# satoutahhaithem/gym

Measured on AMD Instinct MI355X. Metric: strategy-step param GB/s (%HBM/xGMI peak) + ms/outer step, GPT-2 124M, 1-8 GPUs, higher is better.
Workload: dtype f32

## Files before the change

### gym_amd/_lib.py

```python
import ctypes
import os
import threading

_HERE = os.path.dirname(os.path.abspath(__file__))
LIB_PATH = os.environ.get("GYM_AMD_LIB") or os.path.join(_HERE, "_lib", "libgym_amd.so")
HEADER_PATH = os.path.join(os.path.dirname(_HERE), "include", "gym_amd.h")

GA_F32 = 0
GA_BF16 = 1
GA_BF16_REF = 2
GA_LAYOUT_ROWS = 0
GA_LAYOUT_ELEM_MAJOR = 1
GA_MASK_BYTES = 0
GA_MASK_BITS = 1
GA_MASK_TORCH = 2

c_i32, c_i64, c_u32, c_u64, c_f32, c_f64 = (ctypes.c_int32, ctypes.c_int64, ctypes.c_uint32,
                                            ctypes.c_uint64, ctypes.c_float, ctypes.c_double)
c_p = ctypes.c_void_p


class TorchDraw(ctypes.Structure):
    _fields_ = [("table", c_p), ("ntens", c_i32), ("p", c_f32), ("seed", c_u64), ("offset0", c_u64),
                ("offset_step", c_u64), ("seedoff", c_p)]


class DemoTensor(ctypes.Structure):
    _fields_ = [
        ("offset", c_i64), ("payload_off", c_i64),
        ("rows", c_i32), ("cols", c_i32),
        ("n1", c_i32), ("n2", c_i32),
        ("gy", c_i32), ("gx", c_i32),
        ("k", c_i32),
        ("basis1", c_i32), ("basis2", c_i32),
        ("chunk_start", c_i32),
    ]


class DemoRowGroup(ctypes.Structure):
    _fields_ = [("offset", c_i64), ("payload_off", c_i64), ("rows", c_i32), ("k", c_i32)]


SIGNATURES = {
    "ga_abi_version": (c_i32, []),
    "ga_last_error": (ctypes.c_char_p, []),
    "ga_stream_copy": (c_i32, [c_p, c_p, c_i64, c_p]),
    "ga_probe_random_words": (c_i32, [c_p, c_i64, c_i64, c_p, c_i64, c_i32, c_p]),
    "ga_probe_philox": (c_i32, [c_i64, c_p, c_p]),
    "ga_probe_chunk_stream": (c_i32, [c_p, c_p, c_i64, c_i64, c_i32, c_p]),
    "ga_probe_diloco_placement": (c_i32, [c_p, c_i64, c_i64, c_i64, c_p, c_p, c_p]),
    "ga_probe_mean_placement": (c_i32, [c_p, c_i64, c_i64, c_i64, c_p]),
    "ga_probe_adam_placement": (c_i32, [c_p, c_p, c_p, c_p, c_i64, c_i64, c_i64, c_p]),
    "ga_replica_mean": (c_i32, [c_i32, c_p, c_i64, c_i64, c_p, c_i64, c_f32, c_p, c_i64, c_i64, c_p]),
    "ga_diloco_outer": (c_i32, [c_i32, c_p, c_i64, c_i64, c_i64, c_f32, c_p, c_p, c_i32, c_i32, c_f32, c_f32,
                                c_f32, c_f32, c_i32, c_p, c_i64, c_i64, c_p]),
    "ga_diloco_outer_masked": (c_i32, [c_i32, c_p, c_i64, c_i64, c_i64, c_p, c_f32, c_f32, c_p, c_p, c_i32, c_i32,
                                       c_f32, c_f32, c_f32, c_f32, c_i32, c_p, c_i64, c_i64, c_p]),
    "ga_sparta_workspace_bytes": (c_i64, [c_i64]),
    "ga_sparta_gap_table": (None, [c_f64, c_p]),
    "ga_sparta_pack_mask": (c_i32, [c_p, c_i64, c_p, c_p]),
    "ga_sparta_torch_bernoulli_span": (c_i64, []),
    "ga_sparta_torch_draw_bytes": (c_i32, []),
    "ga_sparta_torch_bernoulli": (c_i32, [c_p, c_i32, c_i64, c_f32, c_u64, c_u64, c_u64, c_p, c_p, c_i32, c_p]),
    "ga_sparta_select": (c_i32, [c_i32, c_p, c_i64, c_i64, c_i32, c_i64, c_p, c_i32, c_u64, c_u64, c_f64, c_p, c_i64,
                                 c_i64, c_p, c_p, c_p, c_p, c_p]),
    "ga_sparta_scatter": (c_i32, [c_i32, c_p, c_p, c_p, c_i64, c_f32, c_p, c_i64, c_i64, c_i32, c_p]),
    "ga_sparta_average_local": (c_i32, [c_i32, c_p, c_i64, c_i64, c_i32, c_i64, c_p, c_i32, c_u64, c_u64, c_f64, c_p,
                                        c_i64, c_f32, c_p, c_p, c_i64, c_p, c_p, c_p]),
    "ga_demo_tensor_bytes": (c_i32, []),
    "ga_demo_encode": (c_i32, [c_i32, c_p, c_i32, c_i32, c_p, c_p, c_p, c_p, c_p, c_i64, c_i64, c_f32, c_f32,
                               c_f32, c_p, c_i64, c_i64, c_p]),
    "ga_demo_encode_sym": (c_i32, [c_i32, c_p, c_i32, c_i32, c_p, c_i32, c_p, c_p, c_p, c_p, c_i64, c_i64,
                                   c_f32, c_f32, c_f32, c_p, c_i64, c_i64, c_p]),
    "ga_demo_decode": (c_i32, [c_i32, c_p, c_i32, c_i32, c_p, c_p, c_i64, c_i64, c_i64, c_p, c_p, c_i64,
                               c_i64, c_f32, c_p]),
    "ga_demo_decode_sym": (c_i32, [c_i32, c_p, c_i32, c_i32, c_p, c_i32, c_p, c_p, c_i64, c_i64, c_i64, c_p, c_p,
                                   c_i64, c_i64, c_f32, c_p]),
    "ga_sumsq_partials_count": (c_i32, []),
    "ga_grad_clip_coef": (c_i32, [c_i32, c_p, c_i64, c_i64, c_i64, c_f32, c_p, c_p, c_p]),
    "ga_adam_step": (c_i32, [c_i32, c_p, c_p, c_p, c_p, c_i64, c_i64, c_i64, c_f32, c_f32, c_f32, c_f32, c_f32,
                             c_f32, c_f32, c_f32, c_p, c_p]),
    "ga_replica_gram_workspace_bytes": (c_i64, [c_i64, c_i64]),
    "ga_replica_gram_chain": (c_i32, []),
    "ga_replica_gram": (c_i32, [c_i32, c_p, c_i64, c_i64, c_i64, c_p, c_p, c_p, c_p, c_p]),
    "ga_replica_gram_centered_workspace_bytes": (c_i64, [c_i64, c_i64]),
    "ga_replica_gram_centered": (c_i32, [c_i32, c_p, c_i64, c_i64, c_i64, c_p, c_p, c_p, c_p, c_p, c_p]),
}

_lib = None
_lock = threading.Lock()


class HipLibraryError(RuntimeError):
    pass


def lib():
    global _lib
    if _lib is not None:
        return _lib
    with _lock:
        if _lib is None:
            if not os.path.exists(LIB_PATH):
                raise HipLibraryError(
                    f"{LIB_PATH} is not built: run `make` (or `python __graft_entry__.py`) in the repo root; "
                    "gym_amd has no CPU fallback")
            L = ctypes.CDLL(LIB_PATH)
            for name, (res, args) in SIGNATURES.items():
                fn = getattr(L, name)
                fn.restype = res
                fn.argtypes = args
            if L.ga_demo_tensor_bytes() != ctypes.sizeof(DemoTensor):
                raise HipLibraryError("ga_demo_tensor layout mismatch between libgym_amd.so and gym_amd/_lib.py")
            _lib = L
    return _lib


def check(rc, what):
    if rc != 0:
        msg = lib().ga_last_error().decode(errors="replace")
        raise HipLibraryError(f"{what} failed (code {rc}): {msg}")


def header_symbols(path=HEADER_PATH):
    import re
    txt = open(path).read()
    txt = re.sub(r"/\*.*?\*/", "", txt, flags=re.S)
    return re.findall(r"GA_API\s+[\w\s\*]+?\b(ga_\w+)\s*\(", txt)
```

### gym_amd/csrc/demo_wave.hip

```cpp
#include "ga_common.h"

namespace ga {
namespace dw {

constexpr int kWaves = 8;
constexpr int kThreads = 64 * kWaves;
constexpr int kLd = 65;
constexpr int kCand = 128;
static_assert(2 * (kCand + 64) >= 320, "the fallback top-k keeps its maps in lst[128..319]");

typedef float f32x16 __attribute__((ext_vector_type(16)));

#ifdef GA_DEMO_STAMPS
extern __device__ unsigned long long* g_demo_stamps_w;
#define DW_PH_DECL unsigned long long ph_acc[16] = {}, ph_last = __builtin_amdgcn_s_memtime()
#define DW_PH(i)                                                    \
    do {                                                            \
        const unsigned long long t_ = __builtin_amdgcn_s_memtime(); \
        ph_acc[i] += t_ - ph_last;                                  \
        ph_last = t_;                                               \
    } while (0)
#define DW_CNT(i) (ph_acc[i] += 1)
#define DW_PH_FLUSH()                                                                                       \
    do {                                                                                                    \
        if ((threadIdx.x & 63) == 0) {                                                                      \
            unsigned long long* row_ = g_demo_stamps_w + ((size_t)blockIdx.x * kWaves + (threadIdx.x >> 6)) * 16; \
            for (int i_ = 0; i_ < 16; ++i_) row_[i_] = ph_acc[i_];                                          \
        }                                                                                                   \
    } while (0)
#else
#define DW_PH_DECL do {} while (0)
#define DW_PH(i) do {} while (0)
#define DW_CNT(i) do {} while (0)
#define DW_PH_FLUSH() do {} while (0)
#endif

#define WAVE_LDS_SYNC() asm volatile("" ::: "memory")

__device__ __forceinline__ int lane_id() {
    int t = (int)threadIdx.x;
    asm volatile("" : "+v"(t));
    return t & 63;
}

__device__ __forceinline__ f32x16 zero16() {
    f32x16 a;
#pragma unroll
    for (int r = 0; r < 16; ++r) a[r] = 0.f;
    return a;
}

__device__ __forceinline__ f32x16 mfma(float a, float b, const f32x16& c) {
    return __builtin_amdgcn_mfma_f32_32x32x2f32(a, b, c, 0, 0, 0);
}

__device__ __forceinline__ constexpr int rowmap(int r, int h) { return (r & 3) + 8 * (r >> 2) + 4 * h; }

__device__ __forceinline__ int blk(int h, int q) { return h ? 4 + q : (q < 4 ? q : 8 + q); }

__device__ __forceinline__ int pi_col(int H, int m) { return 4 * blk((m >> 2) & 1, 4 * H + (m >> 3)) + (m & 3); }

__device__ __forceinline__ float basis64(const float* Hb, int i, int d) {
    const float v = Hb[(i < 32 ? i : 63 - i) * kLd + d];
    return (i >= 32 && (d & 1)) ? -v : v;
}

__device__ __forceinline__ uint32_t keyv(float v) { return (__float_as_uint(v) & 0x7fffffffu) + 1u; }

__device__ __forceinline__ int wave_excl_scan128(int v) {
    int r = 0;
#pragma unroll
    for (int b = 0; b < 7; ++b) {
        const uint64_t m = __ballot((v >> b) & 1);
        r += (int)__builtin_amdgcn_mbcnt_hi((uint32_t)(m >> 32), __builtin_amdgcn_mbcnt_lo((uint32_t)m, 0u)) << b;
    }
    return r;
}

__device__ __forceinline__ int wave_sum(int v) {
#pragma unroll
    for (int d = 32; d > 0; d >>= 1) v += __shfl_xor(v, d, 64);
    return v;
}

__device__ __forceinline__ int find_tensor(const ga_demo_tensor* __restrict__ T, int ntens, int tix, int chunk) {
    int lo = tix < 0 ? 0 : tix, hi = ntens - 1;
    while (lo < hi) {
        const int mid = (lo + hi + 1) >> 1;
        if (T[mid].chunk_start <= chunk) lo = mid;
        else hi = mid - 1;
    }
    return lo;
}

__device__ __forceinline__ void decode_wave_priority() {
    const int w = __builtin_amdgcn_readfirstlane((int)threadIdx.x >> 6);
    asm volatile("s_cmp_lt_u32 %0, 4\n\ts_cbranch_scc1 1f\n\ts_setprio 1\n1:" ::"s"(w) : "scc");
}

__device__ __forceinline__ uint32_t rdl(uint32_t v, int j) {
    return (uint32_t)__builtin_amdgcn_readlane((int)v, j);
}

struct ListLDS {
    uint32_t lst[2 * (kCand + 64)];
    uint32_t bm[128];
    uint32_t sm[4];
};

struct WaveLDS : ListLDS {
    float tile[64 * kLd];
};

__device__ __forceinline__ uint32_t lane_off(int s, int q, int l, int h, int stride) {
    return (uint32_t)((s ? 63 - l : l) * stride + 4 * blk(h, q));
}

template <typename T>
__device__ __forceinline__ const T* at_off(const T* pb, uint32_t off) {
    return reinterpret_cast<const T*>(reinterpret_cast<const char*>(pb) + (uint64_t)(uint32_t)(off * (uint32_t)sizeof(T)));
}
template <typename T>
__device__ __forceinline__ T* at_off(T* pb, uint32_t off) {
    return reinterpret_cast<T*>(reinterpret_cast<char*>(pb) + (uint64_t)(uint32_t)(off * (uint32_t)sizeof(T)));
}

template <typename T>
__device__ __forceinline__ void load_rows(const T* pb, int stride, int l, int h, bool vec, int nrows,
                                          float (&o)[2][8][4]) {
    if (vec && nrows == 64) {
#pragma unroll
        for (int s = 0; s < 2; ++s)
#pragma unroll
            for (int q = 0; q < 8; ++q)
                Vec4<T>::unpack(*reinterpret_cast<const typename Vec4<T>::type*>(at_off(pb, lane_off(s, q, l, h, stride))),
                                o[s][q]);
        return;
    }
#pragma unroll
    for (int s = 0; s < 2; ++s) {
        const bool live = (s ? 63 - l : l) < nrows;
#pragma unroll
        for (int q = 0; q < 8; ++q) {
            const T* a = at_off(pb, lane_off(s, q, l, h, stride));
            if (live && vec) {
                Vec4<T>::unpack(*reinterpret_cast<const typename Vec4<T>::type*>(a), o[s][q]);
            } else {
#pragma unroll
                for (int e = 0; e < 4; ++e) o[s][q][e] = live ? Elem<T>::load(a + e) : 0.f;
            }
        }
    }
}

template <typename T>
__device__ __forceinline__ void store_rows(T* pb, int stride, int l, int h, bool vec, int nrows,
                                           const float (&o)[2][8][4]) {
    if (vec && nrows == 64) {
#pragma unroll
        for (int s = 0; s < 2; ++s)
#pragma unroll
            for (int q = 0; q < 8; ++q)
                *reinterpret_cast<typename Vec4<T>::type*>(at_off(pb, lane_off(s, q, l, h, stride))) = Vec4<T>::pack(o[s][q]);
        return;
    }
#pragma unroll
    for (int s = 0; s < 2; ++s) {
        if ((s ? 63 - l : l) >= nrows) continue;
#pragma unroll
        for (int q = 0; q < 8; ++q) {
            T* a = at_off(pb, lane_off(s, q, l, h, stride));
            if (vec) {
                *reinterpret_cast<typename Vec4<T>::type*>(a) = Vec4<T>::pack(o[s][q]);
            } else {
#pragma unroll
                for (int e = 0; e < 4; ++e) Elem<T>::store(a + e, o[s][q][e]);
            }
        }
    }
}
// ... 552 lines not shown
    }
    DW_PH(6);
    {
        const int lane = lane_id(), l = lane & 31, h = lane >> 5;
        f32x16 Tm[2][2];
        row_product(x, Hb, l, h, Tm);
#pragma unroll
        for (int s = 0; s < 2; ++s)
#pragma unroll
            for (int qc = 0; qc < 2; ++qc)
#pragma unroll
                for (int r = 0; r < 16; ++r) {
                    const int i = rowmap(r, h);
                    W.tile[(s ? 63 - i : i) * kLd + 2 * l + qc] = Tm[s][qc][r];
                }
    }
    WAVE_LDS_SYNC();
    {
        const int L = lane_id();
        float* trow = W.tile + L * kLd;
        float yr[64];
#pragma unroll
        for (int t = 0; t < 64; ++t) yr[t] = trow[t];
        uint32_t thr = 0;
        for (int bit = 31; bit >= 0; --bit) {
            const uint32_t cnd = thr | (1u << bit);
            int cl = 0;
#pragma unroll
            for (int t = 0; t < 64; ++t) cl += fabsf(yr[t]) >= __uint_as_float(cnd - 1u) ? 1 : 0;
            if (cl >= k) thr = cnd;
        }
        int gl = 0;
#pragma unroll
        for (int t = 0; t < 64; ++t) gl += keyv(yr[t]) > thr ? 1 : 0;
        int need = k - gl;
        int slot = 0;
        const bool live = L < rows;
        int32_t* oi = pay_idx + (int64_t)L * k;
        float* ov = pay_val + (int64_t)L * k;
#pragma unroll
        for (int t = 0; t < 64; ++t) {
            const uint32_t kv = keyv(yr[t]);
            const bool tie = kv == thr && need > 0;
            const bool s = kv > thr || tie;
            need -= tie ? 1 : 0;
            if (s && live) {
                oi[slot] = t;
                ov[slot] = yr[t];
            }
            slot += s ? 1 : 0;
            trow[t] = s ? yr[t] : 0.f;
        }
    }
    WAVE_LDS_SYNC();
    {
        const int lane = lane_id(), l = lane & 31, h = lane >> 5;
        const int c0 = pi_col(0, l), c1 = pi_col(1, l);
#pragma unroll
        for (int s = 0; s < 2; ++s) {
            const float* yrow = W.tile + (s ? 63 - l : l) * kLd;
            f32x16 r0 = zero16(), r1 = zero16();
#pragma unroll
            for (int t = 0; t < 32; ++t) {
                const int d = 2 * t + h;
                const float yv = yrow[d];
                r0 = mfma(basis64(Hb, c0, d), yv, r0);
                r1 = mfma(basis64(Hb, c1, d), yv, r1);
            }
#pragma unroll
            for (int q = 0; q < 8; ++q)
#pragma unroll
                for (int e = 0; e < 4; ++e) x[s][q][e] -= (q < 4 ? r0 : r1)[4 * (q & 3) + e];
        }
        store_rows(delta, 64, l, h, vec, rows, x);
    }
    WAVE_LDS_SYNC();
    DW_PH(7);
}

template <typename T>
__global__ __launch_bounds__(kThreads) void encode_kernel(
    const ga_demo_tensor* __restrict__ tens, int ntens, int nchunks, const ga_demo_rowgroup* __restrict__ groups,
    int ngroups, const float* __restrict__ F64, T* param0, const T* __restrict__ grad0, T* delta0, int64_t ld,
    int64_t K, float lr, float decay, float wd_factor, int32_t* payload0, int64_t pstride, int64_t M, int ptr_vec) {
    __shared__ float Hb[32 * kLd];
    __shared__ WaveLDS wl[kWaves];
    __shared__ int next_job;
    for (int q = threadIdx.x; q < 32 * 64; q += kThreads) Hb[(q >> 6) * kLd + (q & 63)] = F64[q];
    next_job = 0;
    __syncthreads();
    const int wid = __builtin_amdgcn_readfirstlane((int)threadIdx.x >> 6);
    WaveLDS& W = wl[wid];
    DW_PH_DECL;
    const int64_t n64 = (int64_t)nchunks * K;
    const int64_t stride = (int64_t)gridDim.x * kWaves;
    const int64_t b8 = (int64_t)blockIdx.x * kWaves;
    const int64_t g_total = (int64_t)ngroups * K;
    const uint32_t st = (uint32_t)stride;
    uint32_t nc32 = 0;
#pragma unroll
    for (int w = 0; w < kWaves; ++w)
        if (b8 + w < n64) nc32 += ((uint32_t)(n64 - (b8 + w)) + st - 1u) / st;
    const int64_t nc = nc32;
    const int64_t ng = (int64_t)blockIdx.x < g_total
                           ? ((uint32_t)(g_total - blockIdx.x) + gridDim.x - 1u) / gridDim.x : 0;
    const int64_t nt = nc + ng;
    int tix = -1;
    int64_t last_rep = -1;
    while (true) {
        int tv = 0;
        if (lane_id() == 0) tv = atomicAdd(&next_job, 1);
        const int64_t t = __builtin_amdgcn_readfirstlane(tv);
        if (t >= nt) break;
        const int64_t job = t < ng ? n64 + (int64_t)blockIdx.x + t * gridDim.x
                                   : b8 + ((t - ng) & 7) + ((t - ng) >> 3) * stride;
        if (job < n64) {
            const int64_t rep = job / nchunks;
            const int chunk = (int)(job - rep * nchunks);
            if (rep != last_rep) {
                tix = -1;
                last_rep = rep;
            }
            tix = find_tensor(tens, ntens, tix, chunk);
            const ga_demo_tensor td = tens[tix];
            const int c = chunk - td.chunk_start;
            int32_t* pi = payload0 + rep * pstride + td.payload_off + (int64_t)c * td.k;
            float* pv = reinterpret_cast<float*>(payload0 + rep * pstride + M) + td.payload_off + (int64_t)c * td.k;
            chunk64<T>(td, c, param0 + rep * ld, grad0 + rep * ld, delta0 + rep * ld, pi, pv, lr, decay, wd_factor,
                       ptr_vec, Hb, W
#ifdef GA_DEMO_STAMPS
                       , ph_acc, ph_last
#endif
            );
            DW_CNT(9);
        } else {
            const int64_t j = job - n64;
            const int64_t rep = j / ngroups;
            const int g = (int)(j - rep * ngroups);
            const ga_demo_rowgroup rg = groups[g];
            rowgroup<T>(rg, param0 + rep * ld, grad0 + rep * ld, delta0 + rep * ld,
                        payload0 + rep * pstride + rg.payload_off,
                        reinterpret_cast<float*>(payload0 + rep * pstride + M) + rg.payload_off, lr, decay,
                        wd_factor, ptr_vec, Hb, W
#ifdef GA_DEMO_STAMPS
                        , ph_acc, ph_last
#endif
            );
        }
    }
    DW_PH_FLUSH();
}

template <typename T>
static int launch(const ga_demo_tensor* tens, int32_t ntens, int32_t nchunks, const ga_demo_rowgroup* groups,
                  int32_t ngroups, const float* F64, void* param, const void* grad, void* delta, int64_t K,
                  int64_t ld, float lr, float decay, float wd_factor, int32_t* payload, int64_t pstride, int64_t M,
                  int ptr_vec, hipStream_t stream) {
    static const int cus = [] {
        int dev = 0, n = 0;
        (void)hipGetDevice(&dev);
        (void)hipDeviceGetAttribute(&n, hipDeviceAttributeMultiprocessorCount, dev);
        return n > 0 ? n : 256;
    }();
    auto kern = encode_kernel<T>;
    static const int resident = [&] {
        int per_cu = 0;
        (void)hipOccupancyMaxActiveBlocksPerMultiprocessor(&per_cu, kern, kThreads, 0);
        return (per_cu > 0 ? per_cu : 1) * cus;
    }();
    const int64_t jobs = ((int64_t)nchunks + ngroups) * K;
    const int64_t want = (jobs + kWaves - 1) / kWaves;
    const int grid = (int)(want < resident ? want : resident);
    if (grid <= 0) return GA_OK;
    hipLaunchKernelGGL(kern, dim3(grid), dim3(kThreads), 0, stream, tens, ntens, nchunks, groups, ngroups, F64,
                       (T*)param, (const T*)grad, (T*)delta, ld, K, lr, decay, wd_factor, payload, pstride, M,
                       ptr_vec);
    return GA_OK;
}

constexpr int kMaxSrc = 15;

struct DecLDS {
    float tile[64 * 64];
    uint32_t aux[512];
};

__device__ __forceinline__ int fidx(int row, int col) { return row * 64 + 4 * ((col >> 2) ^ (row & 15)) + (col & 3); }

__device__ __forceinline__ float sgnf(float g) {
    return fabsf(g) > 0.f ? __builtin_copysignf(1.f, g) : 0.f;
}

template <typename T>
using PRaw = typename Vec4<T>::type[16];

template <typename T>
__device__ __forceinline__ void load_coal_raw(const T* pb, int stride, bool vec, int lane, PRaw<T>& o) {
    if (vec) {
#pragma unroll
        for (int i = 0; i < 16; ++i)
            o[i] = *reinterpret_cast<const typename Vec4<T>::type*>(at_off(pb, coal_off(i, lane, stride)));
    } else {
#pragma unroll
        for (int i = 0; i < 16; ++i) {
            float f[4];
#pragma unroll
            for (int e = 0; e < 4; ++e) f[e] = Elem<T>::load(at_off(pb, coal_off(i, lane, stride)) + e);
            o[i] = Vec4<T>::pack(f);
        }
    }
}

template <typename T, bool NTS = false>
__device__ __forceinline__ void store_quad(T* pb, int i, int stride, bool vec, int lane, const float (&f)[4]) {
    T* a = at_off(pb, coal_off(i, lane, stride));
    if (vec) {
        if constexpr (NTS) stream_store(reinterpret_cast<typename Vec4<T>::type*>(a), Vec4<T>::pack(f));
        else store_vec(pb, coal_off(i, lane, stride), Vec4<T>::pack(f));
    } else {
#pragma unroll
        for (int e = 0; e < 4; ++e) Elem<T>::store(a + e, f[e]);
    }
}

template <typename T, bool NTS = false>
__device__ __forceinline__ void sign_update(const float4* tile, T* pr, T* gr, int stride, bool vec, float lr,
                                            int lane, PRaw<T>& raw) {
    if constexpr (sizeof(typename Vec4<T>::type) < 16) {
#pragma unroll
        for (int i = 0; i < 16; ++i) {
            const float4 v = tile[t4((lane >> 4) + 4 * i, lane & 15)];
            float f[4];
            Vec4<T>::unpack(raw[i], f);
            f[0] = fmaf(-lr, v.x, f[0]);
            f[1] = fmaf(-lr, v.y, f[1]);
            f[2] = fmaf(-lr, v.z, f[2]);
            f[3] = fmaf(-lr, v.w, f[3]);
            store_quad(pr, i, stride, vec, lane, f);
        }
        if (gr) {
#pragma unroll
            for (int i = 0; i < 16; ++i) {
                const float4 v = tile[t4((lane >> 4) + 4 * i, lane & 15)];
                const float f[4] = {v.x, v.y, v.z, v.w};
                store_quad<T, NTS>(gr, i, stride, vec, lane, f);
            }
        }
    } else {
#pragma unroll
        for (int i = 0; i < 16; ++i) {
            const float4 v = tile[t4((lane >> 4) + 4 * i, lane & 15)];
            raw[i].x = fmaf(-lr, v.x, raw[i].x);
            raw[i].y = fmaf(-lr, v.y, raw[i].y);
            raw[i].z = fmaf(-lr, v.z, raw[i].z);
            raw[i].w = fmaf(-lr, v.w, raw[i].w);
        }
        if (vec) {
#pragma unroll
            for (int i = 0; i < 16; ++i) *reinterpret_cast<float4*>(at_off(pr, coal_off(i, lane, stride))) = raw[i];
        } else {
// ... 337 lines not shown
        PRaw<T> p0;
        tix = find_tensor(tens, ntens, tix, (int)job);
        ga_demo_tensor td = tens[tix];
        dchunk_entries(td, (int)job - td.chunk_start, payload, pstride, M, S, cur);
        dchunk_params<T>(td, (int)job - td.chunk_start, param, ptr_vec, p0);
        while (true) {
            const int c = (int)job - td.chunk_start;
            const int64_t base = chunk_base(td, c);
            const bool vec = chunk_vec(td, ptr_vec);
            const int cols = td.cols, kc = td.k;
            job += stride;
            if (job < nchunks) {
                tix = find_tensor(tens, ntens, tix, (int)job);
                td = tens[tix];
            }
            dchunk_signs(kc, S, cur, Hb, W, [&] {
                if (job < nchunks) dchunk_entries(td, (int)job - td.chunk_start, payload, pstride, M, S, cur);
            });
            apply_signs<T, NTS>(reinterpret_cast<const float4*>(W.tile), param + base, grad ? grad + base : nullptr,
                                K, ld, cols, vec, 64, lr, lane_id(), p0);
            WAVE_LDS_SYNC();
            if (job >= nchunks) break;
            dchunk_params<T>(td, (int)job - td.chunk_start, param, ptr_vec, p0);
        }
    }
    for (; job < total; job += stride) {
        const ga_demo_rowgroup rg = groups[(int)(job - nchunks)];
        dgroup<T>(rg, payload, pstride, M, S, param, grad, K, ld, lr, ptr_vec, Hb, W);
    }
}

template <typename T, int MS>
static void launch_decode_ms(const ga_demo_tensor* tens, int32_t ntens, int32_t nchunks,
                             const ga_demo_rowgroup* groups, int32_t ngroups, const float* F64,
                             const int32_t* payload, int64_t pstride, int64_t M, int S, void* param, void* grad,
                             int64_t K, int64_t ld, float lr, int ptr_vec, hipStream_t stream) {
    auto kern = decode_kernel<T, MS>;
    static const int resident = [&] {
        int per_cu = 0, dev = 0, cus = 0;
        (void)hipOccupancyMaxActiveBlocksPerMultiprocessor(&per_cu, kern, kThreads, 0);
        (void)hipGetDevice(&dev);
        (void)hipDeviceGetAttribute(&cus, hipDeviceAttributeMultiprocessorCount, dev);
        return (per_cu > 0 ? per_cu : 1) * (cus > 0 ? cus : 256);
    }();
    const int64_t jobs = (int64_t)nchunks + ngroups;
    const int64_t want = (jobs + kWaves - 1) / kWaves;
    const int64_t wr = (int64_t)kWaves * resident;
    int64_t m = S >= 2 ? (8 * jobs + 7 * wr) / (14 * wr)
                       : (6 * jobs + 16 * wr) / (32 * wr);
    if (m < 1) m = 1;
    const int64_t g = resident * m;
    const int grid = (int)(g < want ? g : want);
    if (grid <= 0) return;
    if (S >= 2)
        hipLaunchKernelGGL((decode_kernel<T, MS, true>), dim3(grid), dim3(kThreads), 0, stream, tens, ntens, nchunks,
                           groups, ngroups, F64, payload, pstride, M, S, (T*)param, (T*)grad, K, ld, lr, ptr_vec);
    else
        hipLaunchKernelGGL(kern, dim3(grid), dim3(kThreads), 0, stream, tens, ntens, nchunks, groups, ngroups, F64,
                           payload, pstride, M, S, (T*)param, (T*)grad, K, ld, lr, ptr_vec);
}

template <typename T>
static void launch_decode(const ga_demo_tensor* tens, int32_t ntens, int32_t nchunks, const ga_demo_rowgroup* groups,
                          int32_t ngroups, const float* F64, const int32_t* payload, int64_t pstride, int64_t M,
                          int S, void* param, void* grad, int64_t K, int64_t ld, float lr, int ptr_vec,
                          hipStream_t stream) {
    if (S <= 8)
        launch_decode_ms<T, 8>(tens, ntens, nchunks, groups, ngroups, F64, payload, pstride, M, S, param, grad, K, ld,
                               lr, ptr_vec, stream);
    else
        launch_decode_ms<T, kMaxSrc>(tens, ntens, nchunks, groups, ngroups, F64, payload, pstride, M, S, param, grad,
                                     K, ld, lr, ptr_vec, stream);
}

#ifdef GA_DEMO_STAMPS
__device__ unsigned long long* g_demo_stamps_w;
#endif

}
}

using namespace ga;

#ifdef GA_DEMO_STAMPS
extern "C" GA_API int ga_demo_stamps_set_wave(unsigned long long* buf) {
    return hipMemcpyToSymbol(HIP_SYMBOL(ga::dw::g_demo_stamps_w), &buf, sizeof(buf)) == hipSuccess ? 0 : 2;
}
#endif

extern "C" GA_API int ga_demo_encode_sym(int dtype, const ga_demo_tensor* tensors, int32_t ntensors,
                                         int32_t nchunks, const ga_demo_rowgroup* groups, int32_t ngroups,
                                         const float* F64, void* param, const void* grad, void* delta, int64_t K,
                                         int64_t ld, float lr, float decay, float wd_factor, int32_t* payload,
                                         int64_t payload_stride, int64_t M, hipStream_t stream) {
    clear_error();
    GA_REQUIRE(ntensors >= 0 && nchunks >= 0 && ngroups >= 0 && (nchunks > 0 || ngroups > 0),
               "ga_demo_encode_sym: empty plan (ntensors=%d nchunks=%d ngroups=%d)", ntensors, nchunks, ngroups);
    GA_REQUIRE(nchunks == 0 || (tensors && ntensors >= 1), "ga_demo_encode_sym: no descriptors");
    GA_REQUIRE(ngroups == 0 || groups, "ga_demo_encode_sym: no row groups");
    GA_REQUIRE(F64 && param && grad && delta && payload, "ga_demo_encode_sym: null buffer");
    GA_REQUIRE(K >= 1 && ((int64_t)nchunks + ngroups) * K < (1ll << 31), "ga_demo_encode_sym: K=%lld out of range",
               (long long)K);
    GA_REQUIRE(K == 1 || (ld > 0 && payload_stride >= 2 * M), "ga_demo_encode_sym: bad replica strides");
    const int vb = dtype == GA_F32 ? 16 : 8;
    const int ptr_vec = ((uintptr_t)param % vb == 0) && ((uintptr_t)grad % vb == 0) &&
                        ((uintptr_t)delta % vb == 0) && (K == 1 || ld % 4 == 0);
    switch (dtype) {
        case GA_F32:
            dw::launch<float>(tensors, ntensors, nchunks, groups, ngroups, F64, param, grad, delta, K, ld, lr, decay,
                              wd_factor, payload, payload_stride, M, ptr_vec, stream);
            break;
        case GA_BF16:
            dw::launch<__hip_bfloat16>(tensors, ntensors, nchunks, groups, ngroups, F64, param, grad, delta, K, ld,
                                       lr, decay, wd_factor, payload, payload_stride, M, ptr_vec, stream);
            break;
        default: set_error("ga_demo_encode_sym: unknown dtype %d", dtype); return GA_EINVAL;
    }
    return check_launch("ga_demo_encode_sym");
}

extern "C" GA_API int ga_demo_decode_sym(int dtype, const ga_demo_tensor* tensors, int32_t ntensors,
                                         int32_t nchunks, const ga_demo_rowgroup* groups, int32_t ngroups,
                                         const float* F64, const int32_t* payload, int64_t payload_stride, int64_t M,
                                         int64_t S, void* param, void* grad, int64_t K, int64_t ld, float lr,
                                         hipStream_t stream) {
    clear_error();
    GA_REQUIRE(ntensors >= 0 && nchunks >= 0 && ngroups >= 0 && (nchunks > 0 || ngroups > 0),
               "ga_demo_decode_sym: empty plan (ntensors=%d nchunks=%d ngroups=%d)", ntensors, nchunks, ngroups);
    GA_REQUIRE(nchunks == 0 || (tensors && ntensors >= 1), "ga_demo_decode_sym: no descriptors");
    GA_REQUIRE(ngroups == 0 || groups, "ga_demo_decode_sym: no row groups");
    GA_REQUIRE(F64 && payload && param, "ga_demo_decode_sym: null buffer");
    GA_REQUIRE(S >= 1 && S <= dw::kMaxSrc, "ga_demo_decode_sym: S=%lld sources (1..%d; use ga_demo_decode)",
               (long long)S, dw::kMaxSrc);
    GA_REQUIRE(S == 1 || payload_stride >= 2 * M, "ga_demo_decode_sym: payload_stride < 2*M");
    GA_REQUIRE(K >= 1 && (K == 1 || ld > 0), "ga_demo_decode_sym: bad K=%lld / ld", (long long)K);
    const int vb = dtype == GA_F32 ? 16 : 8;
    const int ptr_vec = ((uintptr_t)param % vb == 0) && (grad == nullptr || (uintptr_t)grad % vb == 0) &&
                        (K == 1 || ld % 4 == 0);
    switch (dtype) {
        case GA_F32:
            dw::launch_decode<float>(tensors, ntensors, nchunks, groups, ngroups, F64, payload, payload_stride, M,
                                     (int)S, param, grad, K, ld, lr, ptr_vec, stream);
            break;
        case GA_BF16:
            dw::launch_decode<__hip_bfloat16>(tensors, ntensors, nchunks, groups, ngroups, F64, payload,
                                              payload_stride, M, (int)S, param, grad, K, ld, lr, ptr_vec, stream);
            break;
        default: set_error("ga_demo_decode_sym: unknown dtype %d", dtype); return GA_EINVAL;
    }
    return check_launch("ga_demo_decode_sym");
}
```

### gym_amd/csrc/ga_common.h

```cpp
#pragma once

#include <hip/hip_runtime.h>
#include <hip/hip_bf16.h>
#include <stdint.h>
#include <stdio.h>
#include <stdarg.h>

#include "../../include/gym_amd.h"

namespace ga {

void set_error(const char* fmt, ...);
void clear_error();

#define GA_REQUIRE(cond, ...)                        \
    do {                                             \
        if (!(cond)) {                               \
            ::ga::set_error(__VA_ARGS__);            \
            return GA_EINVAL;                        \
        }                                            \
    } while (0)

int check_launch(const char* what);

template <typename T> struct Elem;
template <> struct Elem<float> {
    static __device__ __forceinline__ float load(const float* p) { return *p; }
    static __device__ __forceinline__ void store(float* p, float v) { *p = v; }
};
template <> struct Elem<__hip_bfloat16> {
    static __device__ __forceinline__ float load(const __hip_bfloat16* p) {
        return __bfloat162float(*p);
    }
    static __device__ __forceinline__ void store(__hip_bfloat16* p, float v) {
        *p = __float2bfloat16(v);
    }
};

template <typename T> struct Vec4;
template <> struct Vec4<float> {
    using type = float4;
    static __device__ __forceinline__ void unpack(const float4& v, float (&f)[4]) {
        f[0] = v.x; f[1] = v.y; f[2] = v.z; f[3] = v.w;
    }
    static __device__ __forceinline__ float4 pack(const float (&f)[4]) {
        return make_float4(f[0], f[1], f[2], f[3]);
    }
};
template <> struct Vec4<__hip_bfloat16> {
    using type = uint2;
    static __device__ __forceinline__ void unpack(const uint2& v, float (&f)[4]) {
        f[0] = __uint_as_float(v.x << 16);
        f[1] = __uint_as_float(v.x & 0xffff0000u);
        f[2] = __uint_as_float(v.y << 16);
        f[3] = __uint_as_float(v.y & 0xffff0000u);
    }
    static __device__ __forceinline__ uint2 pack(const float (&f)[4]) {
        __hip_bfloat16 b[4];
        for (int i = 0; i < 4; ++i) b[i] = __float2bfloat16(f[i]);
        uint2 r;
        r.x = (uint32_t)__bfloat16_as_ushort(b[0]) | ((uint32_t)__bfloat16_as_ushort(b[1]) << 16);
        r.y = (uint32_t)__bfloat16_as_ushort(b[2]) | ((uint32_t)__bfloat16_as_ushort(b[3]) << 16);
        return r;
    }
};

typedef float ga_f4 __attribute__((ext_vector_type(4)));
typedef unsigned int ga_u2 __attribute__((ext_vector_type(2)));
__device__ __forceinline__ float4 stream_load(const float4* p) {
    const ga_f4 v = __builtin_nontemporal_load(reinterpret_cast<const ga_f4*>(p));
    return make_float4(v.x, v.y, v.z, v.w);
}
__device__ __forceinline__ uint2 stream_load(const uint2* p) {
    const ga_u2 v = __builtin_nontemporal_load(reinterpret_cast<const ga_u2*>(p));
    return make_uint2(v.x, v.y);
}
__device__ __forceinline__ void stream_store(float4* p, const float4& v) {
    ga_f4 w;
    w.x = v.x; w.y = v.y; w.z = v.z; w.w = v.w;
    __builtin_nontemporal_store(w, reinterpret_cast<ga_f4*>(p));
}
__device__ __forceinline__ void stream_store(uint2* p, const uint2& v) {
    ga_u2 w;
    w.x = v.x; w.y = v.y;
    __builtin_nontemporal_store(w, reinterpret_cast<ga_u2*>(p));
}

__device__ __forceinline__ void store_sc1(float4* wg_base, uint32_t idx, const float4& v) {
    const __amdgpu_buffer_rsrc_t r = __builtin_amdgcn_make_buffer_rsrc(wg_base, 0, 0x7fffffff, 0x00020000);
    ga_f4 w;
    w.x = v.x; w.y = v.y; w.z = v.z; w.w = v.w;
    __builtin_amdgcn_raw_buffer_store_b128(w, r, (int)(idx * 16u), 0, 16);
}
__device__ __forceinline__ void store_sc1(uint2* wg_base, uint32_t idx, const uint2& v) {
    const __amdgpu_buffer_rsrc_t r = __builtin_amdgcn_make_buffer_rsrc(wg_base, 0, 0x7fffffff, 0x00020000);
    ga_u2 w;
    w.x = v.x; w.y = v.y;
    __builtin_amdgcn_raw_buffer_store_b64(w, r, (int)(idx * 8u), 0, 16);
}

inline int64_t ceil_div(int64_t a, int64_t b) { return (a + b - 1) / b; }

inline int stream_grid(int64_t work_items, int block) {
    int64_t g = ceil_div(work_items, block);
    if (g > 256 * 16) g = 256 * 16;
    if (g < 1) g = 1;
    return (int)g;
}

}
```

### include/gym_amd.h

```cpp
#ifndef GYM_AMD_H
#define GYM_AMD_H

#include <stdint.h>
#include <hip/hip_runtime_api.h>

#ifdef __cplusplus
extern "C" {
#endif

#define GA_API __attribute__((visibility("default")))

#define GA_OK 0
#define GA_EINVAL 1
#define GA_EHIP 2
#define GA_EUNSUP 3

#define GA_F32 0
#define GA_BF16 1
#define GA_BF16_REF 2

#define GA_LAYOUT_ROWS 0
#define GA_LAYOUT_ELEM_MAJOR 1

#define GA_MASK_BYTES 0
// ... 51 lines not shown
                                  hipStream_t stream);


GA_API int64_t ga_sparta_workspace_bytes(int64_t n);

GA_API void ga_sparta_gap_table(double p, uint64_t* table);

GA_API int ga_sparta_pack_mask(const uint8_t* mask, int64_t n, uint64_t* bits, hipStream_t stream);

GA_API int ga_sparta_torch_draw_bytes(void);

GA_API int64_t ga_sparta_torch_bernoulli_span(void);

GA_API int ga_sparta_torch_bernoulli(const int64_t* table, int32_t ntens, int64_t nblocks, float p,
                                     uint64_t seed, uint64_t offset0, uint64_t offset_step,
                                     const uint64_t* seedoff, void* mask, int mask_format,
                                     hipStream_t stream);

GA_API int ga_sparta_select(int dtype, const void* src, int64_t K, int64_t ld,
                            int layout, int64_t n, const void* mask, int mask_format,
                            uint64_t seed, uint64_t iteration, double p,
                            const int64_t* skip, int64_t nskip, int64_t cap,
                            int32_t* idx, void* vals, int64_t* count, void* work,
                            hipStream_t stream);

GA_API int ga_sparta_scatter(int dtype, const void* vals, const int32_t* idx,
                             const int64_t* count, int64_t cap, float divisor,
                             void* dst, int64_t K, int64_t ld, int layout, hipStream_t stream);

GA_API int ga_sparta_average_local(int dtype, void* reps, int64_t K, int64_t ld, int layout, int64_t n,
                                   const void* mask, int mask_format, uint64_t seed,
                                   uint64_t iteration, double p, const int64_t* skip, int64_t nskip,
                                   float divisor, int32_t* idx, void* vals,
                                   int64_t cap, int64_t* count, void* work, hipStream_t stream);


typedef struct ga_demo_tensor {
    int64_t offset;
    int64_t payload_off;
    int32_t rows, cols;
    int32_t n1, n2;
    int32_t gy, gx;
    int32_t k;
    int32_t basis1, basis2;
    int32_t chunk_start;
} ga_demo_tensor;

GA_API int ga_demo_tensor_bytes(void);


GA_API int ga_demo_encode(int dtype, const ga_demo_tensor* tensors, int32_t ntensors,
                          int32_t nchunks, const float* F, const float* B,
                          void* param, const void* grad, void* delta, int64_t K,
                          int64_t ld, float lr, float decay, float wd_factor,
                          int32_t* payload, int64_t payload_stride, int64_t M,
                          hipStream_t stream);

typedef struct ga_demo_rowgroup {
    int64_t offset;
    int64_t payload_off;
    int32_t rows;
    int32_t k;
} ga_demo_rowgroup;

GA_API int ga_demo_encode_sym(int dtype, const ga_demo_tensor* tensors, int32_t ntensors,
                              int32_t nchunks, const ga_demo_rowgroup* groups, int32_t ngroups,
                              const float* F64, void* param, const void* grad, void* delta,
                              int64_t K, int64_t ld, float lr, float decay, float wd_factor,
                              int32_t* payload, int64_t payload_stride, int64_t M,
                              hipStream_t stream);

GA_API int ga_demo_decode(int dtype, const ga_demo_tensor* tensors, int32_t ntensors,
                          int32_t nchunks, const float* B, const int32_t* payload,
                          int64_t payload_stride, int64_t M, int64_t S, void* param,
                          void* grad, int64_t K, int64_t ld, float lr,
                          hipStream_t stream);

GA_API int ga_demo_decode_sym(int dtype, const ga_demo_tensor* tensors, int32_t ntensors,
                              int32_t nchunks, const ga_demo_rowgroup* groups, int32_t ngroups,
                              const float* F64, const int32_t* payload, int64_t payload_stride,
                              int64_t M, int64_t S, void* param, void* grad, int64_t K, int64_t ld,
                              float lr, hipStream_t stream);


GA_API int ga_sumsq_partials_count(void);

GA_API int ga_grad_clip_coef(int dtype, const void* grad, int64_t K, int64_t ld, int64_t n, float max_norm,
                             float* partials, float* out, hipStream_t stream);

GA_API int ga_adam_step(int dtype, void* param, void* grad, float* exp_avg, float* exp_avg_sq, int64_t K,
                        int64_t ld, int64_t n, float lerp_w, float beta2, float one_m_beta2, float eps,
                        float wd_factor, float l2_wd, float step_size, float bc2_sqrt, const float* clip_coef,
                        hipStream_t stream);


GA_API int64_t ga_replica_gram_workspace_bytes(int64_t K, int64_t n);

GA_API int ga_replica_gram_chain(void);

GA_API int ga_replica_gram(int dtype, const void* src, int64_t K, int64_t ld, int64_t n, double* gram,
                           double* rowsum, double* dist2, void* work, hipStream_t stream);

GA_API int64_t ga_replica_gram_centered_workspace_bytes(int64_t K, int64_t n);

GA_API int ga_replica_gram_centered(int dtype, const void* src, int64_t K, int64_t ld, int64_t n, double* cgram,
                                    double* mdot, double* dsum, double* mstat, void* work, hipStream_t stream);

#ifdef __cplusplus
}
#endif

#endif
```

Baseline: 2508.

## Replace per-block static job split in DeMo encode with a sharded global ticket queue

The sym encode kernel used to hand each block a fixed strided share of chunk and rowgroup jobs, pulled through a block-local LDS counter. It now draws tickets from a global device queue split into 8 shards, with monotonically advancing per-stream host-tracked bases so the counters never need resetting. Blocks steal from other shards when their own is drained, which balances load across blocks. In exchange it adds global atomics per job, host mutex bookkeeping per launch, a refusal to run under graph capture, and test hooks for the queue.

```diff
diff --git a/gym_amd/_lib.py b/gym_amd/_lib.py
--- a/gym_amd/_lib.py
+++ b/gym_amd/_lib.py
@@ -76,6 +76,8 @@
                                c_i64, c_f32, c_p]),
     "ga_demo_decode_sym": (c_i32, [c_i32, c_p, c_i32, c_i32, c_p, c_i32, c_p, c_p, c_i64, c_i64, c_i64, c_p, c_p,
                                    c_i64, c_i64, c_f32, c_p]),
+    "ga_demo_queue_job": (c_i32, [c_u32, c_i32, c_i32, c_i64, c_p, c_p, c_p]),
+    "ga_demo_queue_test_set": (c_i32, [c_u32]),
     "ga_sumsq_partials_count": (c_i32, []),
     "ga_grad_clip_coef": (c_i32, [c_i32, c_p, c_i64, c_i64, c_i64, c_f32, c_p, c_p, c_p]),
     "ga_adam_step": (c_i32, [c_i32, c_p, c_p, c_p, c_p, c_i64, c_i64, c_i64, c_f32, c_f32, c_f32, c_f32, c_f32,
diff --git a/gym_amd/csrc/demo_wave.hip b/gym_amd/csrc/demo_wave.hip
--- a/gym_amd/csrc/demo_wave.hip
+++ b/gym_amd/csrc/demo_wave.hip
@@ -1,4 +1,6 @@
 #include "ga_common.h"
+
+#include <mutex>
 
 namespace ga {
 namespace dw {
@@ -21,6 +23,7 @@
         ph_last = t_;                                               \
     } while (0)
 #define DW_CNT(i) (ph_acc[i] += 1)
+#define DW_WALL(i) (ph_acc[i] = wall_clock64())
 #define DW_PH_FLUSH()                                                                                       \
     do {                                                                                                    \
         if ((threadIdx.x & 63) == 0) {                                                                      \
@@ -32,6 +35,7 @@
 #define DW_PH_DECL do {} while (0)
 #define DW_PH(i) do {} while (0)
 #define DW_CNT(i) do {} while (0)
+#define DW_WALL(i) do {} while (0)
 #define DW_PH_FLUSH() do {} while (0)
 #endif
 
@@ -96,6 +100,72 @@
 __device__ __forceinline__ void decode_wave_priority() {
     const int w = __builtin_amdgcn_readfirstlane((int)threadIdx.x >> 6);
     asm volatile("s_cmp_lt_u32 %0, 4\n\ts_cbranch_scc1 1f\n\ts_setprio 1\n1:" ::"s"(w) : "scc");
+}
+
+constexpr int kQueueSlots = 16;
+constexpr int kQueueShards = 8;
+constexpr int kQueuePad = 1088;
+constexpr int kQueueDevices = 64;
+__device__ uint32_t g_queue[kQueueSlots][kQueueShards][kQueuePad];
+
+struct QueueBases {
+    uint32_t base[kQueueShards];
+};
+
+struct QueueHost {
+    std::mutex mu;
+    struct Dev {
+        QueueBases base[kQueueSlots];
+        hipStream_t stream[kQueueSlots];
+        int used;
+    } dev[kQueueDevices];
+};
+static QueueHost g_queue_host;
+
+__host__ __device__ inline uint32_t queue_shard_jobs(uint32_t jobs, int sh) {
+    return (jobs + (uint32_t)(kQueueShards - 1 - sh)) / (uint32_t)kQueueShards;
+}
+
+template <typename F>
+static int queue_launch(hipStream_t stream, uint32_t jobs, uint32_t waves, F&& launch) {
+    int dev = 0;
+    hipStreamCaptureStatus cap = hipStreamCaptureStatusNone;
+    if (hipGetDevice(&dev) != hipSuccess || dev < 0 || dev >= kQueueDevices) {
+        set_error("DeMo job queue: device %d out of range (< %d)", dev, kQueueDevices);
+        return GA_EINVAL;
+    }
+    if (hipStreamIsCapturing(stream, &cap) != hipSuccess || cap != hipStreamCaptureStatusNone) {
+        (void)hipGetLastError();
+        set_error("DeMo job queue: the stream is under graph capture (a replay would reuse this launch's ticket base)");
+        return GA_EINVAL;
+    }
+    std::lock_guard<std::mutex> lock(g_queue_host.mu);
+    QueueHost::Dev& d = g_queue_host.dev[dev];
+    int slot = 0;
+    while (slot < d.used && d.stream[slot] != stream) ++slot;
+    if (slot == d.used) {
+        if (d.used == kQueueSlots) {
+            if (hipDeviceSynchronize() != hipSuccess) {
+                set_error("DeMo job queue: hipDeviceSynchronize failed");
+                return GA_EHIP;
+            }
+            d.used = slot = 0;
+        }
+        d.stream[d.used++] = stream;
+    }
+    launch(slot, d.base[slot]);
+    if (hipPeekAtLastError() == hipSuccess)
+        for (int sh = 0; sh < kQueueShards; ++sh) d.base[slot].base[sh] += queue_shard_jobs(jobs, sh) + waves;
+    return GA_OK;
+}
+
+__device__ __forceinline__ uint32_t queue_draw(int slot, int shard) {
+    uint32_t tv = 0;
+    if (lane_id() == 0) tv = atomicInc(&g_queue[slot][shard][0], 0xffffffffu);
+    return tv;
+}
+__device__ __forceinline__ uint32_t queue_ticket(uint32_t tv, uint32_t base) {
+    return (uint32_t)__builtin_amdgcn_readfirstlane((int)tv) - base;
 }
 
 __device__ __forceinline__ uint32_t rdl(uint32_t v, int j) {
@@ -814,41 +884,39 @@
 __global__ __launch_bounds__(kThreads) void encode_kernel(
     const ga_demo_tensor* __restrict__ tens, int ntens, int nchunks, const ga_demo_rowgroup* __restrict__ groups,
     int ngroups, const float* __restrict__ F64, T* param0, const T* __restrict__ grad0, T* delta0, int64_t ld,
-    int64_t K, float lr, float decay, float wd_factor, int32_t* payload0, int64_t pstride, int64_t M, int ptr_vec) {
+    int64_t K, float lr, float decay, float wd_factor, int32_t* payload0, int64_t pstride, int64_t M, int ptr_vec,
+    int qslot, QueueBases qb) {
     __shared__ float Hb[32 * kLd];
     __shared__ WaveLDS wl[kWaves];
-    __shared__ int next_job;
+    int shard = (int)(blockIdx.x % kQueueShards);
+    uint32_t tv = queue_draw(qslot, shard);
     for (int q = threadIdx.x; q < 32 * 64; q += kThreads) Hb[(q >> 6) * kLd + (q & 63)] = F64[q];
-    next_job = 0;
     __syncthreads();
     const int wid = __builtin_amdgcn_readfirstlane((int)threadIdx.x >> 6);
     WaveLDS& W = wl[wid];
     DW_PH_DECL;
-    const int64_t n64 = (int64_t)nchunks * K;
-    const int64_t stride = (int64_t)gridDim.x * kWaves;
-    const int64_t b8 = (int64_t)blockIdx.x * kWaves;
-    const int64_t g_total = (int64_t)ngroups * K;
-    const uint32_t st = (uint32_t)stride;
-    uint32_t nc32 = 0;
-#pragma unroll
-    for (int w = 0; w < kWaves; ++w)
-        if (b8 + w < n64) nc32 += ((uint32_t)(n64 - (b8 + w)) + st - 1u) / st;
-    const int64_t nc = nc32;
-    const int64_t ng = (int64_t)blockIdx.x < g_total
-                           ? ((uint32_t)(g_total - blockIdx.x) + gridDim.x - 1u) / gridDim.x : 0;
-    const int64_t nt = nc + ng;
+    DW_WALL(14);
+    const uint32_t jobs = (uint32_t)(((int64_t)nchunks + ngroups) * K);
     int tix = -1;
     int64_t last_rep = -1;
+    int shards_left = kQueueShards;
+    uint32_t qbase = qb.base[shard], sjobs = queue_shard_jobs(jobs, shard);
+    uint32_t t = queue_ticket(tv, qbase);
     while (true) {
-        int tv = 0;
-        if (lane_id() == 0) tv = atomicAdd(&next_job, 1);
-        const int64_t t = __builtin_amdgcn_readfirstlane(tv);
-        if (t >= nt) break;
-        const int64_t job = t < ng ? n64 + (int64_t)blockIdx.x + t * gridDim.x
-                                   : b8 + ((t - ng) & 7) + ((t - ng) >> 3) * stride;
-        if (job < n64) {
-            const int64_t rep = job / nchunks;
-            const int chunk = (int)(job - rep * nchunks);
+        while (t >= sjobs) {
+            if (--shards_left == 0) break;
+            shard = (shard + 1) % kQueueShards;
+            qbase = qb.base[shard];
+            sjobs = queue_shard_jobs(jobs, shard);
+            last_rep = -1;
+            t = queue_ticket(queue_draw(qslot, shard), qbase);
+        }
+        if (shards_left == 0) break;
+        tv = queue_draw(qslot, shard);
+        const DemoJob jb = demo_queue_job(t * kQueueShards + shard, nchunks, ngroups, K);
+        const int64_t rep = jb.rep;
+        if (!jb.is_group) {
+            const int chunk = jb.index;
             if (rep != last_rep) {
                 tix = -1;
                 last_rep = rep;
@@ -866,10 +934,7 @@
             );
             DW_CNT(9);
         } else {
-            const int64_t j = job - n64;
-            const int64_t rep = j / ngroups;
-            const int g = (int)(j - rep * ngroups);
-            const ga_demo_rowgroup rg = groups[g];
+            const ga_demo_rowgroup rg = groups[jb.index];
             rowgroup<T>(rg, param0 + rep * ld, grad0 + rep * ld, delta0 + rep * ld,
                         payload0 + rep * pstride + rg.payload_off,
                         reinterpret_cast<float*>(payload0 + rep * pstride + M) + rg.payload_off, lr, decay,
@@ -879,7 +944,9 @@
 #endif
             );
         }
-    }
+        t = queue_ticket(tv, qbase);
+    }
+    DW_WALL(15);
     DW_PH_FLUSH();
 }
 
@@ -904,10 +971,11 @@
     const int64_t want = (jobs + kWaves - 1) / kWaves;
     const int grid = (int)(want < resident ? want : resident);
     if (grid <= 0) return GA_OK;
-    hipLaunchKernelGGL(kern, dim3(grid), dim3(kThreads), 0, stream, tens, ntens, nchunks, groups, ngroups, F64,
-                       (T*)param, (const T*)grad, (T*)delta, ld, K, lr, decay, wd_factor, payload, pstride, M,
-                       ptr_vec);
-    return GA_OK;
+    return queue_launch(stream, (uint32_t)jobs, (uint32_t)grid * kWaves, [&](int qslot, const QueueBases& qb) {
+        hipLaunchKernelGGL(kern, dim3(grid), dim3(kThreads), 0, stream, tens, ntens, nchunks, groups, ngroups, F64,
+                           (T*)param, (const T*)grad, (T*)delta, ld, K, lr, decay, wd_factor, payload, pstride, M,
+                           ptr_vec, qslot, qb);
+    });
 }
 
 constexpr int kMaxSrc = 15;
@@ -1411,6 +1479,43 @@
 
 using namespace ga;
 
+extern "C" GA_API int ga_demo_queue_job(uint32_t ticket, int32_t nchunks, int32_t ngroups, int64_t K,
+                                        int32_t* is_group, int64_t* rep, int32_t* index) {
+    clear_error();
+    GA_REQUIRE(is_group && rep && index, "ga_demo_queue_job: null output");
+    GA_REQUIRE(nchunks >= 0 && ngroups >= 0 && K >= 1 && ((int64_t)nchunks + ngroups) * K < (1ll << 31) &&
+                   (int64_t)ticket < ((int64_t)nchunks + ngroups) * K,
+               "ga_demo_queue_job: ticket %u outside the job space", ticket);
+    const DemoJob j = demo_queue_job(ticket, nchunks, ngroups, K);
+    *is_group = j.is_group;
+    *rep = j.rep;
+    *index = j.index;
+    return GA_OK;
+}
+
+extern "C" GA_API int ga_demo_queue_test_set(uint32_t value) {
+    clear_error();
+    int dev = 0;
+    GA_REQUIRE(hipGetDevice(&dev) == hipSuccess && dev >= 0 && dev < dw::kQueueDevices,
+               "ga_demo_queue_test_set: no device");
+    std::lock_guard<std::mutex> lock(dw::g_queue_host.mu);
+    if (hipDeviceSynchronize() != hipSuccess) {
+        set_error("ga_demo_queue_test_set: hipDeviceSynchronize failed");
+        return GA_EHIP;
+    }
+    for (int i = 0; i < dw::kQueueSlots; ++i)
+        for (int sh = 0; sh < dw::kQueueShards; ++sh) {
+            dw::g_queue_host.dev[dev].base[i].base[sh] = value;
+            if (hipMemcpyToSymbol(HIP_SYMBOL(ga::dw::g_queue), &value, sizeof(value),
+                                  sizeof(uint32_t) * dw::kQueuePad * ((size_t)i * dw::kQueueShards + sh)) !=
+                hipSuccess) {
+                set_error("ga_demo_queue_test_set: hipMemcpyToSymbol failed");
+                return GA_EHIP;
+            }
+        }
+    return GA_OK;
+}
+
 #ifdef GA_DEMO_STAMPS
 extern "C" GA_API int ga_demo_stamps_set_wave(unsigned long long* buf) {
     return hipMemcpyToSymbol(HIP_SYMBOL(ga::dw::g_demo_stamps_w), &buf, sizeof(buf)) == hipSuccess ? 0 : 2;
@@ -1434,17 +1539,19 @@
     const int vb = dtype == GA_F32 ? 16 : 8;
     const int ptr_vec = ((uintptr_t)param % vb == 0) && ((uintptr_t)grad % vb == 0) &&
                         ((uintptr_t)delta % vb == 0) && (K == 1 || ld % 4 == 0);
+    int rc = GA_OK;
     switch (dtype) {
         case GA_F32:
-            dw::launch<float>(tensors, ntensors, nchunks, groups, ngroups, F64, param, grad, delta, K, ld, lr, decay,
-                              wd_factor, payload, payload_stride, M, ptr_vec, stream);
+            rc = dw::launch<float>(tensors, ntensors, nchunks, groups, ngroups, F64, param, grad, delta, K, ld, lr,
+                                   decay, wd_factor, payload, payload_stride, M, ptr_vec, stream);
             break;
         case GA_BF16:
-            dw::launch<__hip_bfloat16>(tensors, ntensors, nchunks, groups, ngroups, F64, param, grad, delta, K, ld,
-                                       lr, decay, wd_factor, payload, payload_stride, M, ptr_vec, stream);
+            rc = dw::launch<__hip_bfloat16>(tensors, ntensors, nchunks, groups, ngroups, F64, param, grad, delta, K,
+                                            ld, lr, decay, wd_factor, payload, payload_stride, M, ptr_vec, stream);
             break;
         default: set_error("ga_demo_encode_sym: unknown dtype %d", dtype); return GA_EINVAL;
     }
+    if (rc != GA_OK) return rc;
     return check_launch("ga_demo_encode_sym");
 }
 
diff --git a/gym_amd/csrc/ga_common.h b/gym_amd/csrc/ga_common.h
--- a/gym_amd/csrc/ga_common.h
+++ b/gym_amd/csrc/ga_common.h
@@ -99,6 +99,29 @@
     __builtin_amdgcn_raw_buffer_store_b64(w, r, (int)(idx * 8u), 0, 16);
 }
 
+struct DemoJob {
+    int32_t is_group;
+    int32_t index;
+    int64_t rep;
+};
+__host__ __device__ inline DemoJob demo_queue_job(uint32_t ticket, int32_t nchunks, int32_t ngroups, int64_t K) {
+    const uint32_t g_total = (uint32_t)ngroups * (uint32_t)K;
+    DemoJob j;
+    if (ticket < g_total) {
+        const uint32_t rep = ticket / (uint32_t)ngroups;
+        j.is_group = 1;
+        j.index = (int32_t)(ticket - rep * (uint32_t)ngroups);
+        j.rep = rep;
+    } else {
+        const uint32_t c = ticket - g_total;
+        const uint32_t rep = c / (uint32_t)nchunks;
+        j.is_group = 0;
+        j.index = (int32_t)(c - rep * (uint32_t)nchunks);
+        j.rep = rep;
+    }
+    return j;
+}
+
 inline int64_t ceil_div(int64_t a, int64_t b) { return (a + b - 1) / b; }
 
 inline int stream_grid(int64_t work_items, int block) {
diff --git a/include/gym_amd.h b/include/gym_amd.h
--- a/include/gym_amd.h
+++ b/include/gym_amd.h
@@ -157,6 +157,11 @@
                               int64_t M, int64_t S, void* param, void* grad, int64_t K, int64_t ld,
                               float lr, hipStream_t stream);
 
+GA_API int ga_demo_queue_job(uint32_t ticket, int32_t nchunks, int32_t ngroups, int64_t K,
+                             int32_t* is_group, int64_t* rep, int32_t* index);
+
+GA_API int ga_demo_queue_test_set(uint32_t value);
+
 
 GA_API int ga_sumsq_partials_count(void);
 
```

New measurement: 2503. About the same (-0.2%).
